# yangao07/LAMSA

Measured on AMD Instinct MI355X. Metric: aligned Gbase/s, 10 kbp ONT-error reads (12%: sub/ins/del 4% each), -T ont2d vs GRCh37-sized stand-in; inputs resident in HBM when the timed region starts (upload excluded: see pcie_inclusive_*), higher is better.
Workload: dtype int32

## Files before the change

lamsa_amd/csrc/hp_align_api.hip:

```cpp
#include <hip/hip_runtime.h>
#include <algorithm>
#include <atomic>
#include <map>
#include <mutex>
#include <stdlib.h>
#include <string.h>
#include <time.h>
#include "hp_phase.h"
#include "hp_handle.h"
#include "hp_hostprep.h"

using namespace hp;

#ifndef HP_WAVES_PER_SIMD
#define HP_WAVES_PER_SIMD 4
#endif
__global__ __launch_bounds__(64, HP_WAVES_PER_SIMD) void k_align_batch(AlignArgs a)
{
    __shared__ int32_t lds[HP_BOTH_LDS_WORDS];
    const int slot = blockIdx.x;
    for (;;) {
        int u = 0;
        if (wv::leader()) u = atomicAdd(a.counter, 1);
        u = wv::uni(u);
        if (u >= a.n_units) break;
        align_read(a, a.order ? a.order[u] : u, slot, (HP_L int32_t *)lds);
    }
}

#ifndef HP_CHAIN_WAVES_PER_SIMD
#define HP_CHAIN_WAVES_PER_SIMD 4
#endif
#ifndef HP_FILL_WAVES_PER_SIMD
#define HP_FILL_WAVES_PER_SIMD 7
#endif
template <int WORDS, int WPS>
__global__ __launch_bounds__(64, WPS) void k_chain1(const PhaseArgs *ap)
{
    const PhaseArgs &a = *ap;
    __shared__ int32_t lds[WORDS];
    for (;;) {
        int u = 0;
        if (wv::leader()) u = atomicAdd(&a.ctl->q_head[0], 1);
        u = wv::uni(u);
        if (u >= a.n_reads) break;
        phase_chain1(a, a.order ? a.order[u] : u, blockIdx.x, (HP_L int32_t *)lds, WORDS);
    }
    drain_stamp(a, 0);
}
template <int WORDS, int WPS>
__global__ __launch_bounds__(64, WPS) void k_chain2(const PhaseArgs *ap)
{
    const PhaseArgs &a = *ap;
    __shared__ int32_t lds[WORDS];
    for (;;) {
        int u = 0;
        if (wv::leader()) u = atomicAdd(&a.ctl->q_head[2], 1);
        u = wv::uni(u);
        if (u >= a.n_reads) break;
        phase_chain2(a, a.order ? a.order[u] : u, blockIdx.x, (HP_L int32_t *)lds, WORDS);
    }
    drain_stamp(a, 2);
}
typedef void (*ChainKernel)(const PhaseArgs *);
struct ChainShape { ChainKernel k1, k2; int lds_words, waves_per_simd; };
static const ChainShape g_chain_shapes[3] = {
    {k_chain1<HP_CHAIN_LDS_WORDS, HP_CHAIN_WAVES_PER_SIMD>, k_chain2<HP_CHAIN_LDS_WORDS, HP_CHAIN_WAVES_PER_SIMD>, HP_CHAIN_LDS_WORDS, HP_CHAIN_WAVES_PER_SIMD},
    {k_chain1<3392, 3>, k_chain2<3392, 3>, 3392, 3},
    {k_chain1<5120, 2>, k_chain2<5120, 2>, 5120, 2},
};
__global__ __launch_bounds__(64, HP_FILL_WAVES_PER_SIMD) void k_fill(const PhaseArgs *ap, int round)
{
    const PhaseArgs &a = *ap;
    __shared__ int32_t lds[HP_LDS_WORDS];
    int n = 0;
    for (int b = 0; b < PH_NBUCKET; ++b) n += a.ctl->bucket_n[round][b];
    n = wv::uni(n);
    for (;;) {
        int g = 0;
        if (wv::leader()) g = atomicAdd(&a.ctl->q_head[1 + 2 * round], 1);
        g = wv::uni(g);
        if (g >= n) break;
        int b = 0;
        while (b < PH_NBUCKET - 1 && g >= a.ctl->bucket_n[round][b]) { g -= a.ctl->bucket_n[round][b]; ++b; }
        const int u = wv::uni(a.bucket_q[((size_t)round * PH_NBUCKET + b) * a.unit_cap + g]);
        phase_fill(a, round, u, blockIdx.x, (HP_L int32_t *)lds);
    }
    drain_stamp(a, 1 + 2 * round);
}
#ifndef HP_FILLDP_WAVES_PER_SIMD
#define HP_FILLDP_WAVES_PER_SIMD 2
#endif
#ifndef HP_LIST_WAVES_PER_SIMD
#define HP_LIST_WAVES_PER_SIMD 4
#endif
__global__ __launch_bounds__(64, HP_LIST_WAVES_PER_SIMD) void k_filllist(const PhaseArgs *ap, int round)
{
    const PhaseArgs &a = *ap;
    int n = 0;
    for (int b = 0; b < PH_NBUCKET; ++b) n += a.ctl->bucket_n[round][b];
    n = wv::uni(n);
    for (;;) {
        int g = 0;
        if (wv::leader()) g = atomicAdd(&a.ctl->q_head[5], 1);
        g = wv::uni(g);
        if (g >= n) break;
        int b = 0;
        while (b < PH_NBUCKET - 1 && g >= a.ctl->bucket_n[round][b]) { g -= a.ctl->bucket_n[round][b]; ++b; }
        const int u = wv::uni(a.bucket_q[((size_t)round * PH_NBUCKET + b) * a.unit_cap + g]);
        phase_filllist(a, round, u, blockIdx.x, (HP_L int32_t *)nullptr);
    }
}
__global__ __launch_bounds__(64, 2) void k_filldp_small(const PhaseArgs *ap, int round)
{
    __shared__ int32_t lds[HP_LJ_LDS_WORDS(HP_LJ_QSMALL)];
    const PhaseArgs &a = *ap;
    int n = 0;
    for (int b = 0; b < LJ_NBUCKET; ++b) n += ((a.ctl->lj_bucket_n[round][b] < a.lj_cap ? a.ctl->lj_bucket_n[round][b] : a.lj_cap) + 63) >> 6;
    n = wv::uni(n);
    for (;;) {
        int g = 0;
        if (wv::leader()) g = atomicAdd(&a.ctl->q_head[6], 1);
        g = wv::uni(g);
        if (g >= n) break;
        int b = 0;
        for (; b < LJ_NBUCKET - 1; ++b) { const int gb = ((a.ctl->lj_bucket_n[round][b] < a.lj_cap ? a.ctl->lj_bucket_n[round][b] : a.lj_cap) + 63) >> 6; if (g < gb) break; g -= gb; }
        phase_filldp(a, round, b, g * 64, blockIdx.x, (HP_L int32_t *)lds, HP_LJ_QSMALL);
    }
}
__global__ __launch_bounds__(64, HP_WJ_WAVES_PER_SIMD) void k_filldp_wave(const PhaseArgs *ap, int round)
{
    __shared__ int32_t lds[HP_WJ_LDS_WORDS];
    const PhaseArgs &a = *ap;
    int n = 0, n_big = 0;
    for (int b = 0; b < WJ_NBUCKET; ++b) { const int k = a.ctl->wj_bucket_n[round][b] < a.wj_cap ? a.ctl->wj_bucket_n[round][b] : a.wj_cap; if (b < WJ_NBIG) n_big += k; else n += k; }
    n = wv::uni(n); n_big = wv::uni(n_big);
    bool own_big = (int)blockIdx.x < a.n_wjb;
    for (;;) {
        int g = 0;
        const bool big = own_big;
        if (wv::leader()) g = atomicAdd(&a.ctl->q_head[big ? 8 : 7], 1);
        g = wv::uni(g);
        if (g >= (big ? n_big : n)) { if (!big) break; own_big = false; continue; }
// ... 730 lines not shown
```

lamsa_amd/csrc/hp_chain.h:

```cpp
#pragma once
#include "hp_batch.h"
#include "hp_sort.h"

namespace hp {

enum { F_MATCH = 0, F_SPLIT_MATCH = 1, F_MISMATCH = 2, F_MATCH_THD = 2, F_LONG_MISMATCH = 3, F_INSERT = 4, F_DELETE = 5,
       F_CHR_DIF = 6, F_REVERSE = 7, F_UNCONNECT = 8, F_UNMATCH = 9, F_INIT = 20 };
enum { MIN_FLAG = 1, MULTI_FLAG = 2, UNLIMITED_FLAG = 3, WHOLE_FLAG = 4, TRACKED_FLAG = 5 };
enum { L_MERGB = 0, L_NMERG = 1, L_MERGH = 2, L_INTER = 4, L_DUMP = 8 };

HP_INL int score_table(int flag) { return flag <= 3 ? 1 : (flag <= 7 ? -3 : -6); }

#define HP_MAX_SLOTS 16383
#define HP_MAX_HITS_PER_SEED 16383

struct NodeS {
    int64_t pos;
    int32_t chr;
    int32_t slot_j;
    int16_t sid;
    int8_t strand, len_dif8;
    int8_t dp_flag;
    uint8_t son_flag;
    uint8_t match_flag;
// ... 1462 lines not shown
                else if (mf == F_MATCH) F.fr_seed[ns++] = pre;
                else { r.cx.status |= ST_REFEXIT; return false; }
            }
        }
        ++nf;
        F.left_bound[_l] = 0;
        F.line_score[_l] = L.ls[li];
    }
    F.frag_off[line_n] = nf; F.fr_seed_off[nf] = ns;
    F.n = line_n; F.nfrag = nf;
    return true;
}

}
#include "hp_cluster.h"
#include "hp_gaps.h"
namespace hp {

HP_NOINL int lines_pop(ReadCtx &r, NScore &ns, LSet &L, Trig &T, int32_t *_line, const Clusters *C)
{
    int l_i = 0, next_start = 0, line_score = 0, line_NM = 0;
    GapCache gc; gc.n = 0; gc.used = 0; gc.cap = 0; gc.ids = nullptr;
    if (C) gapcache_init(r, gc);
    for (;;) {
        int max_node = ns_pop(ns, &line_score, &line_NM);
        if (max_node < 0) break;
        int32_t *ln = L.pool + next_start;
        T.off[l_i] = T.used; T.cnt[l_i] = 0;
        const int node_i = line_build(r, max_node, ln, _line, &line_score, &line_NM, T, l_i, C, C ? &gc : nullptr);
        if (node_i < 0) return -1;
        { HP_G int32_t *g_ln = (HP_G int32_t *)ln; const int half = node_i / 2;
          for (int k0 = 0; k0 < half; k0 += 64) { WAVE_FOR(l) { const int k = k0 + l; if (k < half) { const int t = g_ln[k], u = g_ln[node_i - k - 1]; g_ln[k] = u; g_ln[node_i - k - 1] = t; } } }
          wv::sync(); }
        L.start[l_i] = next_start; L.len[l_i] = node_i; L.ls[l_i] = L.bs[l_i] = line_score; L.nm[l_i] = line_NM;
        L.mf[l_i] = 0; L.mh[l_i] = 0; L.lb[l_i] = L.rb[l_i] = 0;
        ++l_i; next_start += node_i + 1;
        if (r.cx.status & ST_REFEXIT) return -1;
    }
    return l_i;
}

#ifdef HP_PROF
#define HP_CSTAMP(k) do { const long long now_ = wv::clock(); if (r.prof) r.prof[(k)] += now_ - tc_; tc_ = now_; } while (0)
#else
#define HP_CSTAMP(k) do { } while (0)
#endif

HP_NOINL bool chain_first(ReadCtx &r, FLines &F, FlStore *fs = nullptr)
{
#ifdef HP_PROF
    long long tc_ = wv::clock();
#endif
    const lamsa_hp_para *P = r.cx.P;
    const int seed_out = r.seed_out, H = r.H;
    F.n = 0; F.nfrag = 0;
    int min_n = P->first_loci_thd, min_exist = 0, min_num = 0;
    {
        const HP_G int64_t *g_hoff = (const HP_G int64_t *)r.hit_off;
        for (int i0 = 0; i0 < seed_out; i0 += 64) {
            wv::Lane<int> few;
            WAVE_FOR(l) { const int i = i0 + l; few[l] = i < seed_out && (int)(g_hoff[i + 1] - g_hoff[i]) <= min_n; }
            min_num += __builtin_popcountll(wv::ballot(few));
        }
        min_exist = min_num > 0;
    }
    const bool all_min = (!min_exist || min_num * 3 < seed_out);
#ifdef HP_PROF
    long long tq_ = wv::clock(); if (r.prof) r.prof[56] += tq_ - tc_;
#endif
    if (!r.nodes_ready) {
        for (int base = 0; base < H; base += 64) {
            WAVE_FOR(l) {
                const int k = base + l;
                if (k < H) node_set(r, k, -1, 1, r.h_nm[k], F_MATCH, (all_min || mapn(r, r.n_seed[k]) <= min_n) ? MIN_FLAG : MULTI_FLAG);
            }
        }
        wv::sync();
    }
    r.nodes_ready = false;
#ifdef HP_PROF
    { const long long t2_ = wv::clock(); if (r.prof) r.prof[57] += t2_ - tq_; tq_ = t2_; }
#endif
    if (all_min) min_n = P->per_aln_m;
    const size_t cmark = arena_mark(r.cx.tmp);
    Clusters C;
    bool have_cl = false;
    if (seed_out > 1 && HP_CL_CAP_RT(1) > 0) {
        have_cl = clusters_build(r, C, (HP_L uint64_t *)r.cx.lds, r.cx.lds_words / 2);
        if (!have_cl && (r.cx.status & ST_OVERFLOW)) return false;
    }
    const bool do_me = min_n != P->per_aln_m && seed_out > 1;
    if (do_me && !have_cl) min_extend_all(r, min_n);
#ifdef HP_PROF
    { const long long t2_ = wv::clock(); if (r.prof) { r.prof[58] += t2_ - tq_; r.prof[59] += all_min ? 0 : 1; } }
#endif
    HP_CSTAMP(6);
#if defined(HP_CHAIN_STOP) && HP_CHAIN_STOP == 1
    return true;
#endif
    if (seed_out > 1) {
        bool any_big = false;
        if (!have_cl) dp_update_range(r, hoff(r, 1), H, 0, MIN_FLAG, false, false);
        else {
            const HP_G int32_t *g_cs = (const HP_G int32_t *)C.cs, *g_srt = (const HP_G int32_t *)r.srt;
            HP_G uint8_t *g_big = (HP_G uint8_t *)C.big;
            for (int c0 = 0; c0 < C.n_cl; c0 += 63) {
                wv::Lane<int> csl;
                WAVE_FOR(l) { const int c = c0 + l; csl[l] = c <= C.n_cl ? g_cs[c] : H; }
                const int cn = C.n_cl - c0 < 63 ? C.n_cl - c0 : 63;
                wv::Lane<int> csn = csl;
                WAVE_FOR(l) { const int c = c0 + l + 1; csn[l] = c <= C.n_cl ? g_cs[c] : H; }
                const bool geo32 = (long long)(r.seed_id[seed_out - 1] - r.seed_id[0] + 1) * P->seed_step <= 0x3fffffffll;
                if (geo32 && HP_CL_CAP_RT(1 << 20) >= HP_CLL_MCAP) {
                    const EdgeK K = edge_consts(P);
                    wv::sync();
                    WAVE_FOR(l) { const int n = csn[l] - csl[l]; if (l < cn && n >= 2 && n <= HP_CLL_MCAP) cluster_lane(r, K, C, r.cx.lds + l, csl[l], n, do_me); }
                    wv::sync();
                }
                for (int q = 0; q < cn; ++q) {
                    const int lo = wv::bcast(csl, q), n = wv::bcast(csl, q + 1) - lo;
                    if (n < 2) continue;
                    if (geo32 && HP_CL_CAP_RT(1 << 20) >= HP_CLL_MCAP && n <= HP_CLL_MCAP) continue;
                    if (n <= HP_CL_CAP_RT(r.cx.lds_words / 5) && dp_cluster_lds(r, C, lo, n, do_me)) continue;
                    if (do_me) min_extend_clusters(r, C, lo, lo + n);
                    for (int i0 = 0; i0 < n; i0 += 64) { WAVE_FOR(l) { if (i0 + l < n) g_big[g_srt[lo + i0 + l]] = 1; } }
                    any_big = true;
                }
            }
            wv::sync();
            if (any_big) dp_update_range(r, hoff(r, 1), H, 0, MIN_FLAG, false, false, C.big);
        }
        if (!have_cl) arena_release(r.cx.tmp, cmark);
        if (!build_sons(r, (HP_L uint64_t *)r.cx.lds, r.cx.lds_words / 2)) return false;
    }

    HP_CSTAMP(7);
#if defined(HP_CHAIN_STOP) && HP_CHAIN_STOP == 2
    return true;
#endif
    NScore ns;
    if (!ns_alloc(r.cx, ns, H + 1, 0)) return false;
    ns.min_score_thd = 2;
    track_leaves(r, 0, seed_out - 1, MIN_FLAG, ns);

    HP_CSTAMP(8);
#if defined(HP_CHAIN_STOP) && HP_CHAIN_STOP == 3
    return true;
#endif
    const int o_l = ns.node_n;
    LSet L;
    Trig T;
    if (!lset_alloc(r.cx, L, 2 * H + o_l + 16, o_l)) return false;
    T.cap = 2 * H + 2 * o_l + 16; T.used = 0;
    T.n1 = (int32_t *)arena_alloc(r.cx, sizeof(int32_t) * (size_t)T.cap);
    T.n2 = (int32_t *)arena_alloc(r.cx, sizeof(int32_t) * (size_t)T.cap);
    T.off = (int32_t *)arena_alloc(r.cx, sizeof(int32_t) * (size_t)(o_l + 1));
    T.cnt = (int32_t *)arena_alloc(r.cx, sizeof(int32_t) * (size_t)(o_l + 1));
    int32_t *_line = (int32_t *)arena_alloc(r.cx, sizeof(int32_t) * (size_t)(H + 2));
    if (!T.n1 || !T.n2 || !T.off || !T.cnt || !_line) return false;
    const int l_i = lines_pop(r, ns, L, T, _line, have_cl ? &C : nullptr);
    if (l_i < 0) return false;
    L.n = l_i;
    HP_CSTAMP(9);
#if defined(HP_CHAIN_STOP) && HP_CHAIN_STOP == 4
    return true;
#endif
    LSet S;
    const bool staged = lset_stage(r, L, l_i, S);
    LSet &LL = staged ? S : L;
    const int line_n = set_bound(r, LL, 0, l_i, &T);
    const bool okf = build_flines(r, LL, line_n, F, fs);
    HP_CSTAMP(10);
    if (r.prof) { r.prof[14] = o_l; r.prof[15] = H; }
    return okf;
}

struct RegB { int32_t is_rev, chr; int64_t pos; };
struct Regs {
    int n;
    int32_t *beg, *end; RegB *rb, *re;
    int m;
    int32_t *r_beg, *r_end, *r_bs, *r_bn, *r_es, *r_en;
};

HP_NOINL int multi_line(ReadCtx &r, int left_b, int right_b, const Regs &G, int reg_i, LSet &L)
{
    if (left_b + 1 >= right_b) return 0;
    const lamsa_hp_para *P = r.cx.P;
    const int start = left_b + 1, end = right_b - 1, dp_flag = WHOLE_FLAG;
    nodes_per_init(r, hoff(r, start), hoff(r, end + 1), -1, dp_flag, 1);
    if (start + 1 <= end) dp_update_range(r, hoff(r, start + 1), hoff(r, end + 1), start, dp_flag, false, true);
    const size_t mark = arena_mark(r.cx.tmp);
    NScore ns;
    if (!ns_alloc(r.cx, ns, hoff(r, end + 1) - hoff(r, start) + 1, 0)) return 0;
    ns.min_score_thd = 0;
    track_leaves(r, start, end, dp_flag, ns);
    int l_i = 0, next_start = 0, score = 0, NM = 0;
    for (;;) {
        int rr = ns_pop(ns, &score, &NM);
        if (rr < 0) break;
        int node_i = r.n_node_n[rr] - 1;
        if (l_i >= L.cap || next_start + node_i + 1 > L.pool_cap) { r.cx.status |= ST_OVERFLOW; break; }
        L.start[l_i] = next_start; L.len[l_i] = node_i + 1; L.mf[l_i] = 0; L.mh[l_i] = 0; L.lb[l_i] = L.rb[l_i] = 0;
        next_start += node_i + 1;
        int hit = 0;
        const int64_t expect = (int64_t)((r.n_seed[rr] - left_b) * P->seed_step);
        for (int i = 0; i < G.r_bn[reg_i] && !hit; ++i) {
            const RegB &b = G.re[G.r_bs[reg_i] + i];
            int64_t d = (r.h_pos[rr] - b.pos) - expect; if (d < 0) d = -d;
            if (r.h_chr[rr] == b.chr && d < P->SV_len_thd) hit = 1;
        }
        for (int i = 0; i < G.r_en[reg_i] && !hit; ++i) {
            const RegB &b = G.rb[G.r_es[reg_i] + i];
            int64_t d = (r.h_pos[rr] - b.pos) - expect; if (d < 0) d = -d;
            if (r.h_chr[rr] == b.chr && d < P->SV_len_thd) hit = 1;
        }
        if (hit) { if (score > 1) score += score / 2; else score++; }
        L.ls[l_i] = L.bs[l_i] = score; L.nm[l_i] = NM;
        int32_t *node = L.pool + L.start[l_i];
        while (rr >= 0) {
            if (node_i < 0) { r.cx.status |= ST_REFEXIT; arena_release(r.cx.tmp, mark); return 0; }
            node[node_i--] = rr;
            rr = r.n_from[rr];
        }
        if (node_i >= 0) { r.cx.status |= ST_REFEXIT; arena_release(r.cx.tmp, mark); return 0; }
        ++l_i;
    }
    arena_release(r.cx.tmp, mark);
    return l_i;
}

HP_NOINL bool chain_remain(ReadCtx &r, const Regs &G, FLines &F, FlStore *fs = nullptr)
{
    const lamsa_hp_para *P = r.cx.P;
    const int seed_out = r.seed_out, H = r.H;
    F.n = 0; F.nfrag = 0;
    LSet L, T;
    if (!lset_alloc(r.cx, L, H + 16, H + 1) || !lset_alloc(r.cx, T, H + 16, H + 1)) return false;
    int l_n = 0, next_start = 0;
    for (int i = 0; i < G.m; ++i) {
        const int left_id = (G.r_beg[i] + P->seed_inv - 1) / P->seed_step + 1;
        int right_id = (G.r_end[i] - 1) / P->seed_step + 1;
        if (right_id > r.seed_all) right_id -= 1;
        int left = -2, right = -2;
        for (int j = 0; j < seed_out; ++j) if (r.seed_id[j] >= left_id) { left = j - 1; break; }
        if (left == -2) continue;
        for (int j = seed_out - 1; j >= 0; --j) if (r.seed_id[j] <= right_id) { right = j + 1; break; }
        if (right == -2) continue;
        int l = multi_line(r, left, right, G, i, T);
        if (r.cx.status & ST_REFEXIT) return false;
        T.n = l;
        l = set_bound(r, T, 0, l, nullptr);
        for (int _j = 0; _j < l; ++_j) {
            const int j = T.rank[_j], d = l_n + _j;
            if (d >= L.cap || next_start + T.len[j] > L.pool_cap) { r.cx.status |= ST_OVERFLOW; return false; }
            L.start[d] = next_start; L.len[d] = T.len[j]; L.lb[d] = T.lb[j]; L.rb[d] = T.rb[j]; L.mf[d] = T.mf[j]; L.mh[d] = T.mh[j];
            L.ls[d] = T.ls[j]; L.bs[d] = T.bs[j]; L.nm[d] = T.nm[j];
            for (int k = 0; k < T.len[j]; ++k) L.pool[next_start + k] = T.pool[T.start[j] + k];
            next_start += T.len[j];
            L.rank[d] = d;
        }
        l_n += l;
    }
    L.n = l_n;
    return build_flines(r, L, l_n, F, fs);
}

}
```

lamsa_amd/csrc/hp_phase.h:

```cpp
#pragma once
#include "hp_align.h"
#include "hp_lanedp.h"
#include "hp_wavejob.h"

namespace hp {

struct RdMeta {
    int64_t fl_off[2];
    int32_t fl_n[2], fl_tot[2], fl_nfrag[2];
    int32_t unit_base[2];
    int32_t status;
    int32_t tbases;
    int32_t cells, pairs;
    int32_t cs_words, pad_;
};

struct UnitRec {
    int32_t read, line;
    int64_t out_off;
    int32_t out_len, n_reg;
    int32_t pad[2];
};

enum { PH_NBUCKET = 8, PH_REG_WORDS = 10 };
// ... 21 lines not shown
    char *slab; size_t slab_per_wave;
    int32_t sort_pb, sort_cb;
    const int32_t *order;
    int32_t n_reads;
    long long *prof;
    NodeS *g_nd; int32_t *g_nseed; int32_t *g_sidx;
    RdMeta *meta;
    UnitRec *units; int32_t unit_cap;
    int32_t *bucket_q;
    int32_t *fl_base; int64_t fl_cap;
    int32_t *line_base; int64_t line_cap;
    int32_t *job_base; int64_t job_cap;
    struct LjRec *ljobs; int32_t *lj_bucket; int32_t lj_cap;
    WjRec *wjobs; int32_t *wj_bucket; int32_t wj_cap;
    size_t slab_fill, slab_wj;
    size_t slab_wjb, wjb_off; int32_t n_wjb;
    PhaseCtl *ctl;
};

HP_INL void drain_stamp(const PhaseArgs &a, int k)
{
    if (wv::leader()) { const unsigned long long now = wv::wall(); atomicMax(&a.ctl->t_first_inv[k], ~now); atomicMax(&a.ctl->t_last[k], now); }
}

HP_INL void meta_flag(const PhaseArgs &a, int rd, const ReadCtx &r)
{
    if (wv::leader()) {
        const long long tb = r.t_bases, nc = r.cx.n_cells, np = r.n_pairs, cw = r.cs_words;
        if (r.cx.status) atomicOr(&a.meta[rd].status, r.cx.status);
        if (tb > 0) atomicAdd(&a.meta[rd].tbases, (int)(tb > 0x3fffffffLL ? 0x3fffffffLL : tb));
        if (nc > 0) atomicAdd(&a.meta[rd].cells, (int)(nc > 0x3fffffffLL ? 0x3fffffffLL : nc));
        if (np > 0) atomicAdd(&a.meta[rd].pairs, (int)(np > 0x3fffffffLL ? 0x3fffffffLL : np));
        if (cw > 0) atomicAdd(&a.meta[rd].cs_words, (int)(cw > 0x3fffffffLL ? 0x3fffffffLL : cw));
    }
}

HP_FN void units_push(const PhaseArgs &a, ReadCtx &r, int rd, int round, const FLines &F, const FlStore &fs)
{
    RdMeta &M = a.meta[rd];
    int base = 0;
    if (wv::leader()) base = atomicAdd(&a.ctl->n_units[round], F.n);
    base = wv::uni(base);
    if (base + F.n > a.unit_cap) { r.cx.status |= ST_OVERFLOW; return; }
    M.fl_off[round] = fs.got_off; M.fl_n[round] = F.n; M.fl_tot[round] = fs.got_tot; M.fl_nfrag[round] = F.nfrag; M.unit_base[round] = base;
    const lamsa_hp_para *P = r.cx.P;
    const int tiles = (2 * P->band_w + 1 + 63) / 64;
    for (int j = 0; j < F.n; ++j) {
        const int f0 = F.frag_off[j], f1 = F.frag_off[j + 1];
        const int n_seed = F.fr_seed_off[f1] - F.fr_seed_off[f0];
        const int sa = r.seed_id[r.n_seed[F.fr_seed[F.fr_seed_off[f0]]]], sb = r.seed_id[r.n_seed[F.fr_seed[F.fr_seed_off[f1] - 1]]];
        const int s_lo = sa < sb ? sa : sb, s_hi = sa < sb ? sb : sa;
        long long ext = (long long)(s_lo - 1 + r.seed_all - s_hi) * P->seed_step;
        if (ext < 0) ext = 0;
        const long long cost = ext * tiles * 8 + (long long)n_seed * 64;
        int b = 0;
        for (long long c = cost >> 10; c > 0 && b < PH_NBUCKET - 1; c >>= 1) ++b;
        const int bucket = PH_NBUCKET - 1 - b;
        UnitRec &U = a.units[(size_t)round * a.unit_cap + base + j];
        U.read = rd; U.line = j; U.out_off = 0; U.out_len = 0; U.n_reg = 0;
        int at = 0;
        if (wv::leader()) at = atomicAdd(&a.ctl->bucket_n[round][bucket], 1);
        at = wv::uni(at);
        a.bucket_q[((size_t)round * PH_NBUCKET + bucket) * a.unit_cap + at] = base + j;
    }
}

HP_INL void pers_bind(ReadCtx &r, const PhaseArgs &a, int rd)
{
    const int64_t pb = r.hb + rd;
    r.nd = a.g_nd + pb; r.n_seed = a.g_nseed + pb;
    r.srt = a.g_sidx + 2 * pb; r.rnk = a.g_sidx + 2 * pb + (r.H + 1);
}

#ifdef HP_PROF
#define PH_T0() const long long ph_t0_ = wv::clock()
#define PH_TADD(k) do { if (r.prof) r.prof[k] += wv::clock() - ph_t0_; } while (0)
#define PH_TMID(k, v) do { if (r.prof) { const long long now_ = wv::clock(); r.prof[k] += now_ - v; v = now_; } } while (0)
#else
#define PH_T0() do { } while (0)
#define PH_TADD(k) do { } while (0)
#define PH_TMID(k, v) do { } while (0)
#endif

HP_NOINL void phase_chain1(const PhaseArgs &a, int rd, int wave_slot, HP_L int32_t *lds, int lds_words = HP_CHAIN_LDS_WORDS)
{
#ifdef HP_PROF
    long long ph_t_ = wv::clock();
#endif
    if (a.in.read_skip && a.in.read_skip[rd]) { if (wv::leader()) atomicOr(&a.meta[rd].status, ST_UNSUPPORTED); return; }
    ReadCtx r;
    read_bind(r, a.P, a.ref, a.in, rd, a.slab + (size_t)wave_slot * a.slab_per_wave, a.slab_per_wave, lds, a.prof, lds_words);
    pers_bind(r, a, rd);
    Ctx &cx = r.cx;
    const int H = r.H, c = H + 1;
    int32_t *nm = (int32_t *)arena_alloc(cx, sizeof(int32_t) * 10 * (size_t)c);
    const size_t sort_mark = arena_mark(cx.tmp);
    uint64_t *sort_work = (uint64_t *)arena_alloc(cx, sizeof(uint64_t) * (size_t)c);
    if (nm && sort_work) {
        int32_t *sidx = a.g_sidx + 2 * (r.hb + rd);
        { HP_T0(t_sort_);
        sort_read_hits(r.h_pos, r.h_chr, r.h_strand, H, sidx, sidx + c, sort_work, (HP_L uint64_t *)lds, lds_words / 2, a.sort_pb, a.sort_cb);
        HP_TADD(cx, 46, t_sort_); }
        arena_release(cx.tmp, sort_mark);
        aux_bind(r, nm);
        nodes_fill(r);
        PH_TMID(0, ph_t_);
        FLines F;
        FlStore fs; fs.base = a.fl_base; fs.cap = a.fl_cap; fs.cursor = &a.ctl->fl_cursor; fs.got_off = 0; fs.got_tot = 0;
#if defined(HP_CHAIN_STOP) && HP_CHAIN_STOP == 0
        const bool ok1 = true; F.n = 0; F.nfrag = 0;
#else
        const bool ok1 = chain_first(r, F, &fs);
#endif
        PH_TMID(1, ph_t_);
        if (ok1 && F.n > 0) units_push(a, r, rd, 0, F, fs);
        else if (!ok1 && !(cx.status & (ST_REFEXIT | ST_OVERFLOW))) cx.status |= ST_OVERFLOW;
    }
    meta_flag(a, rd, r);
}

HP_NOINL void phase_fill(const PhaseArgs &a, int round, int u, int wave_slot, HP_L int32_t *lds)
{
    UnitRec &U = a.units[(size_t)round * a.unit_cap + u];
    const int rd = U.read, line = U.line;
    RdMeta &M = a.meta[rd];
    if (*(volatile int32_t *)&M.status & ST_DEAD) return;
    PH_T0();
    ReadCtx r;
    read_bind(r, a.P, a.ref, a.in, rd, a.slab + (size_t)wave_slot * a.slab_fill, a.slab_fill, lds, a.prof, HP_LDS_WORDS);
    pers_bind(r, a, rd);
    Ctx &cx = r.cx;
    FLines F;
    F.n = M.fl_n[round]; F.nfrag = M.fl_nfrag[round];
    flines_bind(F, a.fl_base + M.fl_off[round], F.n, M.fl_tot[round]);
    F.jarena = a.job_base;
    const int cur_cap = 2 * r.L + 512;
    const int out_cap = 64 + 12 * r.L + PH_REG_WORDS * HP_REC_MAX;
    OutBuf o; o.n = 0; o.cap = out_cap;
    o.w = (int32_t *)arena_alloc(cx, sizeof(int32_t) * (size_t)out_cap);
    r.rc_read = (uint8_t *)arena_alloc(cx, (size_t)r.L + 16);
    LineRes *la = (LineRes *)arena_alloc(cx, sizeof(LineRes));
    cig_t *cur_buf = (cig_t *)arena_alloc(cx, sizeof(cig_t) * (size_t)cur_cap);
    cig_t *rec_buf = (cig_t *)arena_alloc(cx, sizeof(cig_t) * (size_t)(cur_cap + 4 * HP_REC_MAX));
    int n_reg = 0;
    if (o.w && r.rc_read && la && cur_buf && rec_buf) {
        const bool ok = fill_line(r, F, line, *la, cur_buf, cur_cap, rec_buf, cur_cap + 4 * HP_REC_MAX);
        if (!ok && !(cx.status & (ST_REFEXIT | ST_OVERFLOW))) cx.status |= ST_OVERFLOW;
        if (ok) {
            out_line(cx, o, *la);
            if (round == 0 && la->tol_score >= 0) {
                Regs G; G.n = 0; G.m = 0;
                const size_t mark = arena_mark(cx.tmp);
                G.beg = (int32_t *)arena_alloc(cx, sizeof(int32_t) * 2 * HP_REC_MAX); G.end = G.beg ? G.beg + HP_REC_MAX : nullptr;
                G.rb = (RegB *)arena_alloc(cx, sizeof(RegB) * 2 * HP_REC_MAX); G.re = G.rb ? G.rb + HP_REC_MAX : nullptr;
                if (G.beg && G.rb) {
                    for (int k = 0; k <= la->cur_res_n; ++k) regs_push(r, G, HP_REC_MAX, la->rec[k]);
                    for (int k = 0; k < G.n; ++k) {
                        out_put(cx, o, G.beg[k]); out_put(cx, o, G.end[k]);
                        out_put(cx, o, G.rb[k].is_rev); out_put(cx, o, G.rb[k].chr); out_put(cx, o, (int32_t)(G.rb[k].pos & 0xffffffffll)); out_put(cx, o, (int32_t)(G.rb[k].pos >> 32));
                        out_put(cx, o, G.re[k].is_rev); out_put(cx, o, G.re[k].chr); out_put(cx, o, (int32_t)(G.re[k].pos & 0xffffffffll)); out_put(cx, o, (int32_t)(G.re[k].pos >> 32));
                    }
                    n_reg = G.n;
                }
                arena_release(cx.tmp, mark);
            }
        }
    }
    if (!(cx.status & (ST_REFEXIT | ST_OVERFLOW))) {
        unsigned long long off = 0;
        if (wv::leader()) off = atomicAdd(&a.ctl->line_cursor, (unsigned long long)o.n);
        off = (unsigned long long)wv::uni64((long long)off);
        if ((int64_t)(off + (unsigned long long)o.n) <= a.line_cap) {
            HP_G int32_t *dst = (HP_G int32_t *)(a.line_base + off);
            const HP_G int32_t *src = (const HP_G int32_t *)o.w;
            wv::sync();
            for (int b = 0; b < o.n; b += 64) { WAVE_FOR(l) { const int i = b + l; if (i < o.n) dst[i] = src[i]; } }
            U.out_off = (int64_t)off; U.out_len = o.n; U.n_reg = n_reg;
        } else cx.status |= ST_OVERFLOW;
    }
    PH_TADD(round == 0 ? 2 : 4);
    meta_flag(a, rd, r);
}


struct LjRec { int64_t qaddr, tk, slot; int32_t rd; uint16_t tlen; uint8_t qlen; int8_t type_comp; };
enum { LJ_NCLS = HP_LJ_QSMALL / 16, LJ_NBUCKET = 2 * LJ_NCLS };
HP_INL int lj_bucket_of(int type, int qlen)
{
    const int cls = (qlen > 0 ? qlen - 1 : 0) >> 4;
    return (type == 1 ? 0 : LJ_NCLS) + (LJ_NCLS - 1 - cls);
}

struct EndGeo { int s, read_start, read_len, chr; int64_t start0; int32_t ref_len; };
HP_INL bool end_geo(const ReadCtx &r, const FLines &F, int line, int strand, bool head, EndGeo &G)
{
    const lamsa_hp_para *P = r.cx.P;
    const int f0 = F.frag_off[line], fl = F.frag_off[line + 1] - 1;
    const int lb = strand == 1 ? F.left_bound[line] : r.seed_all + 1 - F.right_bound[line];
    const int rb = strand == 1 ? F.right_bound[line] : r.seed_all + 1 - F.left_bound[line];
    const int s_first = F.fr_seed[F.fr_seed_off[f0]], s_last = F.fr_seed[F.fr_seed_off[fl + 1] - 1];
    int64_t ref_start;
// ... 258 lines not shown
        if (l < cnt && bq[l] >= 0) {
            const LjRec R = a.ljobs[bq[l]];
            LaneJob J;
            const int comp = (R.type_comp >> 4) & 1, type = R.type_comp & 15;
            J.q = (const HP_G uint8_t *)(a.in.read_seq + R.qaddr); J.qs = comp ? -1 : 1; J.qcomp = comp; J.qlen = R.qlen; J.pac = (const HP_G uint8_t *)a.ref.pac; J.tk = R.tk; J.ts = 1; J.tlen = R.tlen;
            J.z = (HP_G uint8_t *)zbuf; J.zl = l; J.zs = qcap; J.cells = 0; J.row = lds + l; J.qrow = (HP_L uint8_t *)(lds + (qcap + 2) * 64) + l; J.rev = 0;
            lj_stage_query(J);
            LCig out, Lc, Rc;
            out.c = cbuf + (size_t)l * 3 * HP_LJ_CIG; out.n = 0; Lc.c = out.c + HP_LJ_CIG; Lc.n = 0; Rc.c = Lc.c + HP_LJ_CIG; Rc.n = 0;
            if (type == 1) lj_bi_extend(P, J, 100, 100, Lc, Rc, out);
            else lj_global(P, J, P->del_gapo, P->del_gape, P->ins_gapo, P->ins_gape, P->band_w, &out);
            nw[l] = out.n; rdl[l] = R.rd; cel[l] = (int)J.cells; slotl[l] = R.slot | ((long long)R.tlen << 48);
        }
    }
    wv::Lane<int> pre = nw;
    wv::scan_add_excl(pre);
    const int total = wv::reduce_sum(nw);
    unsigned long long base = 0;
    if (wv::leader()) base = atomicAdd(&a.ctl->job_cursor, (unsigned long long)total);
    base = (unsigned long long)wv::uni64((long long)base);
    if ((int64_t)(base + (unsigned long long)total) > a.job_cap) return;
    WAVE_FOR(l) {
        if (l < cnt && bq[l] >= 0) {
            const cig_t *src = cbuf + (size_t)l * 3 * HP_LJ_CIG;
            int32_t *dst = a.job_base + base + pre[l];
            for (int k = 0; k < nw[l]; ++k) dst[k] = src[k];
            int32_t *slot = a.fl_base + (slotl[l] & 0xffffffffffffll);
            slot[0] = (int32_t)(base + pre[l]); slot[1] = nw[l]; slot[2] = (int32_t)(slotl[l] >> 48); slot[3] = 1;
            if (cel[l] > 0) atomicAdd(&a.meta[rdl[l]].cells, cel[l]);
        }
    }
    wv::sync();
}

#ifdef HP_WJ_NOINL
HP_NOINL
#else
HP_INL
#endif
void phase_wavejob(const PhaseArgs &a, int round, int g, bool big, int wave_slot, HP_L int32_t *lds)
{
    const int b1 = big ? WJ_NBIG : WJ_NBUCKET;
    int b = big ? 0 : WJ_NBIG;
    for (; b < b1 - 1; ++b) { const int nb = a.ctl->wj_bucket_n[round][b] < a.wj_cap ? a.ctl->wj_bucket_n[round][b] : a.wj_cap; if (g < nb) break; g -= nb; }
    const int ji = wv::uni(a.wj_bucket[(size_t)b * a.wj_cap + g]);
    if (ji < 0) return;
    const WjRec R = a.wjobs[ji];
    const int rd = wv::uni(R.rd), type = wv::uni(R.type_comp) & 15, comp = (wv::uni(R.type_comp) >> 4) & 1;
    const int qs = (wv::uni(R.type_comp) >> 5) & 1 ? -1 : 1, ts = (wv::uni(R.type_comp) >> 6) & 1 ? -1 : 1;
    const int qlen = wv::uni(R.qlen), tlen = wv::uni(R.tlen);
    if (*(volatile int32_t *)&a.meta[rd].status & ST_DEAD) return;
    Ctx cx;
    cx.P = &a.P; cx.lds = lds; cx.lds_words = HP_WJ_LDS_WORDS; cx.status = 0; cx.n_cells = 0; cx.lds_epoch = 0; cx.prof = a.prof ? a.prof + (size_t)rd * 64 : nullptr;
    cx.prof_dp = a.prof ? a.prof + ((size_t)a.n_reads + 1 + rd) * 64 : nullptr;
    if (big) arena_init(cx.tmp, a.slab + a.wjb_off + (size_t)wave_slot * a.slab_wjb, a.slab_wjb);
    else arena_init(cx.tmp, a.slab + (size_t)wave_slot * a.slab_wj, a.slab_wj);
    CigV out;
    if (!cig_alloc(cx, out, qlen + tlen + 64)) return;
    WjOut o;
    const lamsa_hp_para *P = &a.P;
    const bool ok = wj_run(cx, a.in.read_seq, a.ref.pac, type, comp, wv::uni64(R.qaddr), qs, qlen, wv::uni64(R.tk), ts, tlen,
                           P->band_w, type == WJ_BI ? 100 : P->seed_len * P->match, out, o);
    if (cx.n_cells > 0 && wv::leader()) { atomicAdd(&a.meta[rd].cells, (int)(cx.n_cells > 0x3fffffffLL ? 0x3fffffffLL : cx.n_cells)); atomicAdd(&a.ctl->wj_cells, (unsigned long long)cx.n_cells); }
    if (!ok) return;
    unsigned long long base = 0;
    if (wv::leader()) base = atomicAdd(&a.ctl->job_cursor, (unsigned long long)out.n);
    base = (unsigned long long)wv::uni64((long long)base);
    if ((int64_t)(base + (unsigned long long)out.n) > a.job_cap) return;
    {
        HP_G int32_t *dst = (HP_G int32_t *)(a.job_base + base);
        const HP_G cig_t *src = (const HP_G cig_t *)out.c;
        for (int b0 = 0; b0 < out.n; b0 += 64) { WAVE_FOR(l) { const int i = b0 + l; if (i < out.n) dst[i] = src[i]; } }
        HP_G int32_t *slot = (HP_G int32_t *)(a.fl_base + wv::uni64(R.slot));
        WAVE_FOR(l) {
            if (type == WJ_BI || type == WJ_GLOBAL) { if (l < 4) slot[l] = l == 0 ? (int32_t)base : (l == 1 ? out.n : (l == 2 ? tlen : 1)); }
            else if (l < 8) slot[l] = l == 0 ? (int32_t)base : (l == 1 ? out.n : (l == 2 ? o.reflen : (l == 3 ? o.readlen : (l == 4 ? 1 : 0))));
        }
    }
    if (wv::leader()) atomicAdd(&a.ctl->wj_bytes, (unsigned long long)(qlen + (tlen + 3) / 4 + 4 * out.n + 32));
    HP_STAT(9);
    wv::sync();
}

HP_NOINL void phase_chain2(const PhaseArgs &a, int rd, int wave_slot, HP_L int32_t *lds, int lds_words = HP_CHAIN_LDS_WORDS)
{
    RdMeta &M = a.meta[rd];
    if (M.status & ST_DEAD) return;
    PH_T0();
    ReadCtx r;
    read_bind(r, a.P, a.ref, a.in, rd, a.slab + (size_t)wave_slot * a.slab_per_wave, a.slab_per_wave, lds, a.prof, lds_words);
    pers_bind(r, a, rd);
    Ctx &cx = r.cx;
    const int H = r.H, c = H + 1;
    int32_t *nm = (int32_t *)arena_alloc(cx, sizeof(int32_t) * 10 * (size_t)c);
    const int reg_cap = 256;
    Regs G; G.n = 0; G.m = 0;
    G.beg = (int32_t *)arena_alloc(cx, sizeof(int32_t) * 2 * (size_t)reg_cap); G.end = G.beg + reg_cap;
    G.rb = (RegB *)arena_alloc(cx, sizeof(RegB) * 2 * (size_t)reg_cap); G.re = G.rb + reg_cap;
    G.r_beg = (int32_t *)arena_alloc(cx, sizeof(int32_t) * 6 * (size_t)(reg_cap + 2));
    G.r_end = G.r_beg + (reg_cap + 2); G.r_bs = G.r_end + (reg_cap + 2); G.r_bn = G.r_bs + (reg_cap + 2); G.r_es = G.r_bn + (reg_cap + 2); G.r_en = G.r_es + (reg_cap + 2);
    if (nm && G.beg && G.rb && G.r_beg) {
        aux_bind(r, nm);
        for (int j = 0; j < M.fl_n[0]; ++j) {
            const UnitRec &U = a.units[M.unit_base[0] + j];
            const int32_t *w = a.line_base + U.out_off + (U.out_len - PH_REG_WORDS * U.n_reg);
            for (int k = 0; k < U.n_reg; ++k, w += PH_REG_WORDS) {
                if (G.n >= reg_cap) { cx.status |= ST_OVERFLOW; break; }
                const int g = G.n++;
                G.beg[g] = w[0]; G.end[g] = w[1];
                G.rb[g].is_rev = w[2]; G.rb[g].chr = w[3]; G.rb[g].pos = (int64_t)(((unsigned long long)(unsigned)w[5] << 32) | (unsigned)w[4]);
                G.re[g].is_rev = w[6]; G.re[g].chr = w[7]; G.re[g].pos = (int64_t)(((unsigned long long)(unsigned)w[9] << 32) | (unsigned)w[8]);
            }
        }
        wv::sync();
        if (!(cx.status & ST_OVERFLOW)) {
            regs_remain(r, G, a.P.seed_len, r.L);
            FLines F;
            FlStore fs; fs.base = a.fl_base; fs.cap = a.fl_cap; fs.cursor = &a.ctl->fl_cursor; fs.got_off = 0; fs.got_tot = 0;
            const bool ok2 = chain_remain(r, G, F, &fs);
            if (ok2 && F.n > 0) units_push(a, r, rd, 1, F, fs);
            else if (!ok2 && !(cx.status & (ST_REFEXIT | ST_OVERFLOW))) cx.status |= ST_OVERFLOW;
        }
    }
    PH_TADD(3);
    meta_flag(a, rd, r);
}

HP_NOINL void phase_publish(const PhaseArgs &a, int rd)
{
    const RdMeta &M = a.meta[rd];
    const int st = M.status;
    const bool dead = (st & ST_DEAD) != 0;
    int n_words = 3;
    if (!dead)
        for (int round = 0; round < 2; ++round)
            for (int j = 0; j < M.fl_n[round]; ++j) { const UnitRec &U = a.units[(size_t)round * a.unit_cap + M.unit_base[round] + j]; n_words += U.out_len - PH_REG_WORDS * U.n_reg; }
    unsigned long long off = 0;
    if (wv::leader()) off = atomicAdd(a.out.cursor, (unsigned long long)n_words);
    off = (unsigned long long)wv::uni64((long long)off);
    if ((int64_t)(off + (unsigned long long)n_words) <= a.out.stream_cap) {
        HP_G int32_t *dst = (HP_G int32_t *)(a.out.stream + off);
        dst[0] = st; dst[1] = dead ? 0 : M.fl_n[0]; dst[2] = dead ? 0 : M.fl_n[1];
        int at = 3;
        if (!dead)
            for (int round = 0; round < 2; ++round)
                for (int j = 0; j < M.fl_n[round]; ++j) {
                    const UnitRec &U = a.units[(size_t)round * a.unit_cap + M.unit_base[round] + j];
                    const int n = U.out_len - PH_REG_WORDS * U.n_reg;
                    const HP_G int32_t *src = (const HP_G int32_t *)(a.line_base + U.out_off);
                    for (int b = 0; b < n; b += 64) { WAVE_FOR(l) { const int i = b + l; if (i < n) dst[at + i] = src[i]; } }
                    at += n;
                }
        a.out.read_out_off[rd] = (int64_t)off; a.out.read_out_len[rd] = n_words;
    } else { a.out.read_out_off[rd] = -1; a.out.read_out_len[rd] = 0; }
    a.out.read_status[rd] = st;
    if (a.out.read_tbases) a.out.read_tbases[rd] = M.tbases;
    if (a.out.read_work) { a.out.read_work[4 * rd] = M.cells; a.out.read_work[4 * rd + 1] = M.pairs; a.out.read_work[4 * rd + 2] = M.cs_words; a.out.read_work[4 * rd + 3] = 0; }
}

HP_INL void publish_diag(const PhaseArgs &a)
{
    if (a.out.diag && wv::leader()) {
        for (int k = 0; k < 4; ++k) { a.out.diag[2 * k] = ~a.ctl->t_first_inv[k]; a.out.diag[2 * k + 1] = a.ctl->t_last[k]; }
        a.out.diag[8] = (unsigned long long)a.ctl->n_units[0]; a.out.diag[9] = (unsigned long long)a.ctl->n_units[1];
        a.out.diag[10] = a.ctl->fl_cursor; a.out.diag[11] = a.ctl->line_cursor;
        a.out.diag[12] = (unsigned long long)(a.ctl->wj_n[0] + a.ctl->wj_n[1]); a.out.diag[13] = a.ctl->wj_bytes; a.out.diag[14] = (unsigned long long)(a.ctl->lj_n[0] + a.ctl->lj_n[1]);
        a.out.diag[15] = a.ctl->job_cursor; a.out.diag[16] = a.ctl->wj_cells;
    }
}

}
```

Baseline: 3.591.

## Move chain-phase read context and local structs out of private stack into LDS/arena

The chain kernels now hold the per-wave ReadCtx in LDS when the extra 512 bytes fit the occupancy budget, and otherwise at the head of the wave's global slab. Large local structs (Clusters, NScore, LSet, Trig, FLines, Regs) are allocated from the per-read arena instead of living on the stack. The intent is to remove scratch (private memory) spills and stack frames in these non-inlined functions. In exchange, accesses to these structs go through generic pointers to LDS or global memory, and the slab usable by the arena shrinks by the context block.

```diff
diff --git a/lamsa_amd/csrc/hp_align_api.hip b/lamsa_amd/csrc/hp_align_api.hip
--- a/lamsa_amd/csrc/hp_align_api.hip
+++ b/lamsa_amd/csrc/hp_align_api.hip
@@ -38,13 +38,15 @@
 __global__ __launch_bounds__(64, WPS) void k_chain1(const PhaseArgs *ap)
 {
     const PhaseArgs &a = *ap;
-    __shared__ int32_t lds[WORDS];
+    constexpr bool ctx_lds = ph_ctx_in_lds(WORDS, WPS);
+    __shared__ alignas(16) int32_t lds[WORDS + (ctx_lds ? PH_CTX_BYTES / 4 : 0)];
+    ReadCtx &r = *(ctx_lds ? (ReadCtx *)(lds + WORDS) : (ReadCtx *)(a.slab + (size_t)blockIdx.x * a.slab_per_wave));
     for (;;) {
         int u = 0;
         if (wv::leader()) u = atomicAdd(&a.ctl->q_head[0], 1);
         u = wv::uni(u);
         if (u >= a.n_reads) break;
-        phase_chain1(a, a.order ? a.order[u] : u, blockIdx.x, (HP_L int32_t *)lds, WORDS);
+        phase_chain1(a, a.order ? a.order[u] : u, blockIdx.x, (HP_L int32_t *)lds, WORDS, r);
     }
     drain_stamp(a, 0);
 }
@@ -52,13 +54,15 @@
 __global__ __launch_bounds__(64, WPS) void k_chain2(const PhaseArgs *ap)
 {
     const PhaseArgs &a = *ap;
-    __shared__ int32_t lds[WORDS];
+    constexpr bool ctx_lds = ph_ctx_in_lds(WORDS, WPS);
+    __shared__ alignas(16) int32_t lds[WORDS + (ctx_lds ? PH_CTX_BYTES / 4 : 0)];
+    ReadCtx &r = *(ctx_lds ? (ReadCtx *)(lds + WORDS) : (ReadCtx *)(a.slab + (size_t)blockIdx.x * a.slab_per_wave));
     for (;;) {
         int u = 0;
         if (wv::leader()) u = atomicAdd(&a.ctl->q_head[2], 1);
         u = wv::uni(u);
         if (u >= a.n_reads) break;
-        phase_chain2(a, a.order ? a.order[u] : u, blockIdx.x, (HP_L int32_t *)lds, WORDS);
+        phase_chain2(a, a.order ? a.order[u] : u, blockIdx.x, (HP_L int32_t *)lds, WORDS, r);
     }
     drain_stamp(a, 2);
 }
diff --git a/lamsa_amd/csrc/hp_chain.h b/lamsa_amd/csrc/hp_chain.h
--- a/lamsa_amd/csrc/hp_chain.h
+++ b/lamsa_amd/csrc/hp_chain.h
@@ -1568,8 +1568,11 @@
     { const long long t2_ = wv::clock(); if (r.prof) r.prof[57] += t2_ - tq_; tq_ = t2_; }
 #endif
     if (all_min) min_n = P->per_aln_m;
+    struct Loc { Clusters C; NScore ns; LSet L, S; Trig T; };
+    Loc *loc = (Loc *)arena_alloc(r.cx, sizeof(Loc));
+    if (!loc) return false;
     const size_t cmark = arena_mark(r.cx.tmp);
-    Clusters C;
+    Clusters &C = loc->C;
     bool have_cl = false;
     if (seed_out > 1 && HP_CL_CAP_RT(1) > 0) {
         have_cl = clusters_build(r, C, (HP_L uint64_t *)r.cx.lds, r.cx.lds_words / 2);
@@ -1624,7 +1627,7 @@
 #if defined(HP_CHAIN_STOP) && HP_CHAIN_STOP == 2
     return true;
 #endif
-    NScore ns;
+    NScore &ns = loc->ns;
     if (!ns_alloc(r.cx, ns, H + 1, 0)) return false;
     ns.min_score_thd = 2;
     track_leaves(r, 0, seed_out - 1, MIN_FLAG, ns);
@@ -1634,8 +1637,8 @@
     return true;
 #endif
     const int o_l = ns.node_n;
-    LSet L;
-    Trig T;
+    LSet &L = loc->L;
+    Trig &T = loc->T;
     if (!lset_alloc(r.cx, L, 2 * H + o_l + 16, o_l)) return false;
     T.cap = 2 * H + 2 * o_l + 16; T.used = 0;
     T.n1 = (int32_t *)arena_alloc(r.cx, sizeof(int32_t) * (size_t)T.cap);
@@ -1651,7 +1654,7 @@
 #if defined(HP_CHAIN_STOP) && HP_CHAIN_STOP == 4
     return true;
 #endif
-    LSet S;
+    LSet &S = loc->S;
     const bool staged = lset_stage(r, L, l_i, S);
     LSet &LL = staged ? S : L;
     const int line_n = set_bound(r, LL, 0, l_i, &T);
@@ -1677,7 +1680,9 @@
     nodes_per_init(r, hoff(r, start), hoff(r, end + 1), -1, dp_flag, 1);
     if (start + 1 <= end) dp_update_range(r, hoff(r, start + 1), hoff(r, end + 1), start, dp_flag, false, true);
     const size_t mark = arena_mark(r.cx.tmp);
-    NScore ns;
+    NScore *nsp = (NScore *)arena_alloc(r.cx, sizeof(NScore));
+    if (!nsp) return 0;
+    NScore &ns = *nsp;
     if (!ns_alloc(r.cx, ns, hoff(r, end + 1) - hoff(r, start) + 1, 0)) return 0;
     ns.min_score_thd = 0;
     track_leaves(r, start, end, dp_flag, ns);
@@ -1721,7 +1726,9 @@
     const lamsa_hp_para *P = r.cx.P;
     const int seed_out = r.seed_out, H = r.H;
     F.n = 0; F.nfrag = 0;
-    LSet L, T;
+    LSet *lt = (LSet *)arena_alloc(r.cx, 2 * sizeof(LSet));
+    if (!lt) return false;
+    LSet &L = lt[0], &T = lt[1];
     if (!lset_alloc(r.cx, L, H + 16, H + 1) || !lset_alloc(r.cx, T, H + 16, H + 1)) return false;
     int l_n = 0, next_start = 0;
     for (int i = 0; i < G.m; ++i) {
diff --git a/lamsa_amd/csrc/hp_phase.h b/lamsa_amd/csrc/hp_phase.h
--- a/lamsa_amd/csrc/hp_phase.h
+++ b/lamsa_amd/csrc/hp_phase.h
@@ -127,21 +127,29 @@
 #define PH_TMID(k, v) do { } while (0)
 #endif
 
-HP_NOINL void phase_chain1(const PhaseArgs &a, int rd, int wave_slot, HP_L int32_t *lds, int lds_words = HP_CHAIN_LDS_WORDS)
+enum { PH_CTX_BYTES = 512 };
+static_assert(sizeof(ReadCtx) <= PH_CTX_BYTES, "the read context must fit its per-wave block");
+constexpr bool ph_ctx_in_lds(int words, int waves_per_simd)
+{
+    return 4 * waves_per_simd * (((size_t)words * 4 + PH_CTX_BYTES + 511) / 512 * 512) <= 160 * 1024;
+}
+struct ChainOut { FLines F; FlStore fs; };
+
+HP_NOINL void phase_chain1(const PhaseArgs &a, int rd, int wave_slot, HP_L int32_t *lds, int lds_words, ReadCtx &r)
 {
 #ifdef HP_PROF
     long long ph_t_ = wv::clock();
 #endif
     if (a.in.read_skip && a.in.read_skip[rd]) { if (wv::leader()) atomicOr(&a.meta[rd].status, ST_UNSUPPORTED); return; }
-    ReadCtx r;
-    read_bind(r, a.P, a.ref, a.in, rd, a.slab + (size_t)wave_slot * a.slab_per_wave, a.slab_per_wave, lds, a.prof, lds_words);
+    read_bind(r, a.P, a.ref, a.in, rd, a.slab + (size_t)wave_slot * a.slab_per_wave + PH_CTX_BYTES, a.slab_per_wave - PH_CTX_BYTES, lds, a.prof, lds_words);
     pers_bind(r, a, rd);
     Ctx &cx = r.cx;
     const int H = r.H, c = H + 1;
+    ChainOut *co = (ChainOut *)arena_alloc(cx, sizeof(ChainOut));
     int32_t *nm = (int32_t *)arena_alloc(cx, sizeof(int32_t) * 10 * (size_t)c);
     const size_t sort_mark = arena_mark(cx.tmp);
     uint64_t *sort_work = (uint64_t *)arena_alloc(cx, sizeof(uint64_t) * (size_t)c);
-    if (nm && sort_work) {
+    if (co && nm && sort_work) {
         int32_t *sidx = a.g_sidx + 2 * (r.hb + rd);
         { HP_T0(t_sort_);
         sort_read_hits(r.h_pos, r.h_chr, r.h_strand, H, sidx, sidx + c, sort_work, (HP_L uint64_t *)lds, lds_words / 2, a.sort_pb, a.sort_cb);
@@ -150,8 +158,8 @@
         aux_bind(r, nm);
         nodes_fill(r);
         PH_TMID(0, ph_t_);
-        FLines F;
-        FlStore fs; fs.base = a.fl_base; fs.cap = a.fl_cap; fs.cursor = &a.ctl->fl_cursor; fs.got_off = 0; fs.got_tot = 0;
+        FLines &F = co->F;
+        FlStore &fs = co->fs; fs.base = a.fl_base; fs.cap = a.fl_cap; fs.cursor = &a.ctl->fl_cursor; fs.got_off = 0; fs.got_tot = 0;
 #if defined(HP_CHAIN_STOP) && HP_CHAIN_STOP == 0
         const bool ok1 = true; F.n = 0; F.nfrag = 0;
 #else
@@ -162,6 +170,12 @@
         else if (!ok1 && !(cx.status & (ST_REFEXIT | ST_OVERFLOW))) cx.status |= ST_OVERFLOW;
     }
     meta_flag(a, rd, r);
+}
+
+HP_FN void phase_chain1(const PhaseArgs &a, int rd, int wave_slot, HP_L int32_t *lds, int lds_words = HP_CHAIN_LDS_WORDS)
+{
+    ReadCtx r;
+    phase_chain1(a, rd, wave_slot, lds, lds_words, r);
 }
 
 HP_NOINL void phase_fill(const PhaseArgs &a, int round, int u, int wave_slot, HP_L int32_t *lds)
@@ -586,19 +600,21 @@
     wv::sync();
 }
 
-HP_NOINL void phase_chain2(const PhaseArgs &a, int rd, int wave_slot, HP_L int32_t *lds, int lds_words = HP_CHAIN_LDS_WORDS)
+HP_NOINL void phase_chain2(const PhaseArgs &a, int rd, int wave_slot, HP_L int32_t *lds, int lds_words, ReadCtx &r)
 {
     RdMeta &M = a.meta[rd];
     if (M.status & ST_DEAD) return;
     PH_T0();
-    ReadCtx r;
-    read_bind(r, a.P, a.ref, a.in, rd, a.slab + (size_t)wave_slot * a.slab_per_wave, a.slab_per_wave, lds, a.prof, lds_words);
+    read_bind(r, a.P, a.ref, a.in, rd, a.slab + (size_t)wave_slot * a.slab_per_wave + PH_CTX_BYTES, a.slab_per_wave - PH_CTX_BYTES, lds, a.prof, lds_words);
     pers_bind(r, a, rd);
     Ctx &cx = r.cx;
     const int H = r.H, c = H + 1;
+    ChainOut *co = (ChainOut *)arena_alloc(cx, sizeof(ChainOut));
+    Regs *gp = (Regs *)arena_alloc(cx, sizeof(Regs));
+    if (!co || !gp) { meta_flag(a, rd, r); return; }
     int32_t *nm = (int32_t *)arena_alloc(cx, sizeof(int32_t) * 10 * (size_t)c);
     const int reg_cap = 256;
-    Regs G; G.n = 0; G.m = 0;
+    Regs &G = *gp; G.n = 0; G.m = 0;
     G.beg = (int32_t *)arena_alloc(cx, sizeof(int32_t) * 2 * (size_t)reg_cap); G.end = G.beg + reg_cap;
     G.rb = (RegB *)arena_alloc(cx, sizeof(RegB) * 2 * (size_t)reg_cap); G.re = G.rb + reg_cap;
     G.r_beg = (int32_t *)arena_alloc(cx, sizeof(int32_t) * 6 * (size_t)(reg_cap + 2));
@@ -619,8 +635,8 @@
         wv::sync();
         if (!(cx.status & ST_OVERFLOW)) {
             regs_remain(r, G, a.P.seed_len, r.L);
-            FLines F;
-            FlStore fs; fs.base = a.fl_base; fs.cap = a.fl_cap; fs.cursor = &a.ctl->fl_cursor; fs.got_off = 0; fs.got_tot = 0;
+            FLines &F = co->F;
+            FlStore &fs = co->fs; fs.base = a.fl_base; fs.cap = a.fl_cap; fs.cursor = &a.ctl->fl_cursor; fs.got_off = 0; fs.got_tot = 0;
             const bool ok2 = chain_remain(r, G, F, &fs);
             if (ok2 && F.n > 0) units_push(a, r, rd, 1, F, fs);
             else if (!ok2 && !(cx.status & (ST_REFEXIT | ST_OVERFLOW))) cx.status |= ST_OVERFLOW;
@@ -628,6 +644,12 @@
     }
     PH_TADD(3);
     meta_flag(a, rd, r);
+}
+
+HP_FN void phase_chain2(const PhaseArgs &a, int rd, int wave_slot, HP_L int32_t *lds, int lds_words = HP_CHAIN_LDS_WORDS)
+{
+    ReadCtx r;
+    phase_chain2(a, rd, wave_slot, lds, lds_words, r);
 }
 
 HP_NOINL void phase_publish(const PhaseArgs &a, int rd)
```

Result: faster. 3.796, median of 6 (+5.7%).
